# OpenDriveLab/Vista

Measured on AMD Instinct MI355X. Metric: denoise steps/sec, 25-frame 576x1024 latent, 50-step EDM @ 1/2/4/8 GPU, higher is better.
Workload: dtype bf16; 1 GPU; 1xMI355X single GPU: 25x576x1024 (latent 25x4x72x128), 50-step EulerEDM, VanillaCFG 2.5 (N=50 images per UNet call), bf16, random-init 1.65B VideoUNet, synthetic latents; frames=25, cfg_images_per_call=50, sampler=EulerEDM s_churn=0, 50-step schedule, parallelism=single GPU

## Files before the change

include/vista_hip.h:

```cpp
#ifndef VISTA_HIP_H
#define VISTA_HIP_H
#include <stdint.h>
#ifdef __cplusplus
extern "C" {
#endif

enum { VK_AMODE_DENSE = 0, VK_AMODE_CONV3X3 = 1, VK_AMODE_TEMPORAL3 = 2, VK_AMODE_CONV3D = 3 };
enum { VK_EPI_LINEAR = 0, VK_EPI_GEGLU = 1, VK_EPI_TRANS = 2 };

typedef struct VkGemmDesc {
    const void* A;
    const void* Wt;
    void* out;
    const float* bias;
    const float* rowvec;
    const void* res1;
    const void* res2;
    int32_t M, N, K;
    int32_t lda, ldc, ld_res1, ld_res2, ldv, rows_per_vec;
    float alpha, beta;
    int32_t amode, epi, out_f32;
    int32_t H, Wd, Cin, Hout, Wout, stride, ups;
    int32_t T, S;
    int32_t tile_cfg;
// ... 46 lines not shown
int vk_ff_fused_bf16(const VkGemmDesc* geglu, const VkGemmDesc* out_proj, void* stream);
int vk_ff_fused_rowstat_parts(void);

int vk_groupnorm_silu_fp8(const void* x1, const void* x2, void* y8, float* scale_out, const float* gamma, const float* beta, float* stats_ws,
                          int32_t n_img, int32_t S, int32_t C1, int32_t C2, int32_t frames_per_group, float eps, int32_t silu, void* stream);

int vk_layernorm_quant_fp8(const void* x, void* q, float* scale, const float* gamma, const float* beta, int32_t rows, int32_t C, float eps,
                           void* stream);

int vk_quantize_rows_fp8(const void* x, void* q, float* scale, int32_t M, int32_t K, int64_t ldx, int64_t ldq, void* stream);

int vk_attn_spatial_bf16(const void* q, const void* k, const void* vt, void* o, int32_t n_img, int32_t heads,
                         int32_t S, int32_t ldq, int32_t ldk, int32_t ldo, float scale, void* stream);

int vk_attn_spatial_qkv_bf16(const void* q, const void* k, const void* v, void* o, int32_t n_img, int32_t heads,
                             int32_t S, int32_t ldq, int32_t ldk, int32_t ldv, int32_t ldo, float scale, void* stream);

int vk_attn_spatial_qkv_log2_bf16(const void* q, const void* k, const void* v, void* o, int32_t n_img, int32_t heads,
                                  int32_t S, int32_t ldq, int32_t ldk, int32_t ldv, int32_t ldo, void* stream);

int vk_attn_small_bf16(const void* qkv, void* o, int32_t n_img, int32_t heads, int32_t S, int32_t D, int32_t ld, int32_t k_off,
                       int32_t v_off, int32_t ldo, float scale, void* stream);

int vk_clip_preprocess_patches(const float* img, void* out, int32_t n_img, int32_t H, int32_t W, int32_t out_hw, int32_t patch, int32_t ldo,
                               float sigma_y, float sigma_x, int32_t ks_y, int32_t ks_x, const float* mean3, const float* std3, void* stream);

int vk_attn_spatial_fp8qk(const void* q8, const void* k8, const void* q_scales, const void* k_scales, const void* v, void* o, void* o8,
                          void* o_scales, int32_t n_img, int32_t heads, int32_t S, int32_t ldq8, int32_t ldk8, int32_t ldqs, int32_t ldks,
                          int32_t ldv, int32_t ldo, int32_t ldo8, int32_t ldos, float scale, void* stream);

int vk_attn_temporal_bf16(const void* qkv, void* o, int32_t B, int32_t T, int32_t S, int32_t heads, int32_t ld,
                          int32_t k_off, int32_t v_off, int32_t ldo, float scale, void* stream);

int vk_softmax_rows_f32_bf16(const float* x, void* y, int64_t rows, int32_t cols, int64_t ldx, int64_t ldy, void* stream);

int vk_groupnorm_silu_bf16(const void* x, void* y, const float* gamma, const float* beta, float* stats_ws,
                           int32_t n_img, int32_t S, int32_t C, int32_t frames_per_group, float eps, int32_t silu,
                           void* stream);

int vk_groupnorm_stats_bf16(const void* x, float* sums, float* partial_ws, int32_t n_img, int32_t S, int32_t C,
                            int32_t frames_per_group, void* stream);
int vk_groupnorm_apply_bf16(const void* x, void* y, const float* gamma, const float* beta, const float* sums, int32_t n_img,
                            int32_t S, int32_t C, int32_t frames_per_group, float count, float eps, int32_t silu, void* stream);
int vk_groupnorm_finalize_partials(float* partial, float* sums, int32_t n_img, int32_t nchunks, int32_t frames_per_group, void* stream);
int vk_groupnorm_fold_max(void);
int vk_groupnorm_apply_partials_bf16(const void* x, void* y, const float* gamma, const float* beta, const float* partial, int32_t n_img,
                                     int32_t S, int32_t C, int32_t nchunks, int32_t frames_per_group, float count, float eps, int32_t silu,
                                     void* stream);

int vk_layernorm_bf16(const void* x, void* y, void* sum_out, const float* gamma, const float* beta,
                      const float* addvec, int32_t rows, int32_t C, int32_t rows_per_vec, int32_t ldv, float eps,
                      void* stream);

int vk_rowstats_bf16(const void* x, float* stats, int32_t rows, int32_t C, int64_t ldx, void* stream);

int vk_groupnorm_silu_cat_bf16(const void* x1, const void* x2, void* y, const float* gamma, const float* beta, float* stats_ws,
                               int32_t n_img, int32_t S, int32_t C1, int32_t C2, int32_t frames_per_group, float eps, int32_t silu,
                               void* stream);

int vk_concat_channels_bf16(const void* a, const void* b, void* out, int64_t rows, int32_t C1, int32_t C2, void* stream);

int vk_nchw_to_tokens_bf16(const float* x, void* out, int32_t n_img, int32_t C, int32_t HW, int32_t Cpad, void* stream);
int vk_tokens_to_nchw_f32(const float* x, float* out, int32_t n_img, int32_t C, int32_t HW, int32_t ldx, void* stream);

int vk_timestep_embedding_bf16(const float* t, void* out, int32_t n, int32_t dim, float max_period, void* stream);
int vk_timestep_embedding_f32(const float* t, float* out, int32_t n, int32_t dim, float max_period, void* stream);
// ... 93 lines not shown
```

vista_amd/_lib.py:

```python
import ctypes as C
import os

_HERE = os.path.dirname(os.path.abspath(__file__))
ACT_DTYPE = os.environ.get("VISTA_ACT_DTYPE", "bf16").lower()
if ACT_DTYPE not in ("bf16", "fp16"):
    raise ValueError(f"VISTA_ACT_DTYPE must be 'bf16' or 'fp16', not {ACT_DTYPE!r}")
CURRENT = ACT_DTYPE
_LIB_FILES = {"bf16": "libvista_hip.so", "fp16": "libvista_hip_f16.so"}
LIB_PATH = os.environ.get("VISTA_HIP_LIB") or os.path.join(_HERE, "lib", _LIB_FILES[ACT_DTYPE])


def lib_path(dtype_name):
    return LIB_PATH if dtype_name == ACT_DTYPE else os.path.join(_HERE, "lib", _LIB_FILES[dtype_name])


_vp = C.c_void_p
_i32 = C.c_int32
_i64 = C.c_int64
_f32 = C.c_float


class VkFp8Args(C.Structure):
    _fields_ = [("a_scale", _vp), ("w_scale", _vp), ("k_real", _i32), ("a_mx", _vp), ("ld_mx", _i32), ("mx_out", _vp), ("ld_mx_out", _i32),
                ("a_scale_rows", _i32)]
# ... 43 lines not shown

class VkStrokeSet(C.Structure):
    _fields_ = [("stroke_begin", _i32), ("stroke_count", _i32)]


class VkStrokePlan(C.Structure):
    _fields_ = [("n_sets", _i32), ("n_strokes", _i32), ("n_segments", _i32), ("reserved", _i32), ("set", VkStrokeSet * VK_OVERLAY_MAX_SETS),
                ("stroke", VkStroke * VK_OVERLAY_MAX_STROKES), ("seg", VkStrokeSegment * VK_OVERLAY_MAX_SEGMENTS)]


ABI_VERSION = 9

SIGNATURES = {
    "vk_gemm_bf16": [C.POINTER(VkGemmDesc), _vp],
    "vk_gemm_rowstat_parts": [C.POINTER(VkGemmDesc)],
    "vk_gemm_tile_choice": [C.POINTER(VkGemmDesc)],
    "vk_gemm_tail_split": [C.POINTER(VkGemmDesc)],
    "vk_gemm_gnstat_fit": [C.POINTER(VkGemmDesc)],
    "vk_gemm_fp8": [C.POINTER(VkGemmDesc), _vp, _vp, _i32, _vp],
    "vk_gemm_fp8_mx": [C.POINTER(VkGemmDesc), C.POINTER(VkFp8Args), _vp],
    "vk_gemm_fp8_rowstat_parts": [C.POINTER(VkGemmDesc)],
    "vk_ff_fused_bf16": [C.POINTER(VkGemmDesc), C.POINTER(VkGemmDesc), _vp],
    "vk_ff_fused_rowstat_parts": [],
    "vk_layernorm_quant_fp8": [_vp, _vp, _vp, _vp, _vp, _i32, _i32, _f32, _vp],
    "vk_groupnorm_silu_fp8": [_vp, _vp, _vp, _vp, _vp, _vp, _vp, _i32, _i32, _i32, _i32, _i32, _f32, _i32, _vp],
    "vk_quantize_rows_fp8": [_vp, _vp, _vp, _i32, _i32, _i64, _i64, _vp],
    "vk_attn_spatial_bf16": [_vp, _vp, _vp, _vp, _i32, _i32, _i32, _i32, _i32, _i32, _f32, _vp],
    "vk_attn_spatial_qkv_bf16": [_vp, _vp, _vp, _vp, _i32, _i32, _i32, _i32, _i32, _i32, _i32, _f32, _vp],
    "vk_attn_spatial_qkv_log2_bf16": [_vp, _vp, _vp, _vp, _i32, _i32, _i32, _i32, _i32, _i32, _i32, _vp],
    "vk_attn_spatial_fp8qk": [_vp, _vp, _vp, _vp, _vp, _vp, _vp, _vp, _i32, _i32, _i32, _i32, _i32, _i32, _i32, _i32, _i32, _i32, _i32, _f32, _vp],
    "vk_attn_small_bf16": [_vp, _vp, _i32, _i32, _i32, _i32, _i32, _i32, _i32, _i32, _f32, _vp],
    "vk_clip_preprocess_patches": [_vp, _vp, _i32, _i32, _i32, _i32, _i32, _i32, _f32, _f32, _i32, _i32, C.POINTER(_f32), C.POINTER(_f32), _vp],
    "vk_attn_temporal_bf16": [_vp, _vp, _i32, _i32, _i32, _i32, _i32, _i32, _i32, _i32, _f32, _vp],
    "vk_softmax_rows_f32_bf16": [_vp, _vp, _i64, _i32, _i64, _i64, _vp],
    "vk_groupnorm_silu_bf16": [_vp, _vp, _vp, _vp, _vp, _i32, _i32, _i32, _i32, _f32, _i32, _vp],
    "vk_groupnorm_stats_bf16": [_vp, _vp, _vp, _i32, _i32, _i32, _i32, _vp],
    "vk_groupnorm_apply_bf16": [_vp, _vp, _vp, _vp, _vp, _i32, _i32, _i32, _i32, _f32, _f32, _i32, _vp],
    "vk_groupnorm_finalize_partials": [_vp, _vp, _i32, _i32, _i32, _vp],
    "vk_groupnorm_fold_max": [],
    "vk_groupnorm_apply_partials_bf16": [_vp, _vp, _vp, _vp, _vp, _i32, _i32, _i32, _i32, _i32, _f32, _f32, _i32, _vp],
    "vk_layernorm_bf16": [_vp, _vp, _vp, _vp, _vp, _vp, _i32, _i32, _i32, _i32, _f32, _vp],
    "vk_rowstats_bf16": [_vp, _vp, _i32, _i32, _i64, _vp],
    "vk_groupnorm_silu_cat_bf16": [_vp, _vp, _vp, _vp, _vp, _vp, _i32, _i32, _i32, _i32, _i32, _f32, _i32, _vp],
    "vk_concat_channels_bf16": [_vp, _vp, _vp, _i64, _i32, _i32, _vp],
    "vk_nchw_to_tokens_bf16": [_vp, _vp, _i32, _i32, _i32, _i32, _vp],
    "vk_tokens_to_nchw_f32": [_vp, _vp, _i32, _i32, _i32, _i32, _vp],
    "vk_timestep_embedding_bf16": [_vp, _vp, _i32, _i32, _f32, _vp],
    "vk_timestep_embedding_f32": [_vp, _vp, _i32, _i32, _f32, _vp],
    "vk_emb_combine": [_vp, _vp, _vp, _vp, _vp, _vp, _i32, _i32, _vp],
    "vk_silu_f32_to_bf16": [_vp, _vp, _i64, _vp],
    "vk_cast_f32_to_bf16": [_vp, _vp, _i64, _vp],
    "vk_sampler_prepare": [_vp, _vp, _vp, _vp, _vp, _vp, _i32, _i32, _i32, _f32, _i32, _vp],
    "vk_sampler_update": [_vp, _vp, _vp, _i32, _i32, _i32, _f32, _f32, _f32, _f32, _vp],
    "vk_denoiser_combine": [_vp, _vp, _vp, _vp, _vp, _i32, _i32, _vp],
    "vk_cfg_combine": [_vp, _vp, _vp, _i32, _i32, _vp],
    "vk_euler_step": [_vp, _vp, _vp, _vp, _vp, _i32, _i32, _vp],
    "vk_mask_replace": [_vp, _vp, _vp, _vp, _i32, _i32, _vp],
    "vk_scale_rows": [_vp, _vp, _vp, _i32, _i32, _vp],
    "vk_gaussian_sample": [_vp, _vp, _vp, _i32, _i32, _i32, _f32, _vp],
    "vk_ensemble_variance_sum": [_vp, _vp, _vp, _i32, _i64, _vp],
    "vk_lanczos_resize_u8": [_vp, _vp, _vp, _vp, _vp, _i32, _vp, _vp, _i32, _vp, _i32, _i32, _i32, _i32, _i32, _i32, _i32, _i32, _i32, _vp],
    "vk_frames_to_u8": [_vp, _vp, _i32, _i32, _i32, _i32, _i32, _i32, _vp],
    "vk_ensemble_frame_stats": [_vp, _vp, _vp, _vp, _i32, _i32, _i32, _i32, _vp],
    "vk_candidate_frame_stats": [_vp, _vp, _vp, _vp, _vp, _vp, _i32, _i32, _i32, _i32, _i32, _i32, _vp],
    "vk_heat_overlay_u8": [_vp, _vp, _vp, _i32, _i32, _i32, _i32, _f32, _f32, _vp],
    "vk_frame_fidelity_ws_bytes": [_i32, _i32],
# ... 43 lines not shown
```

vista_amd/build.py:

```python
import os
import subprocess
import sys

ROOT = os.path.dirname(os.path.abspath(__file__))
REPO = os.path.dirname(ROOT)
CSRC = os.path.join(ROOT, "csrc")
LIBDIR = os.path.join(ROOT, "lib")
LIB = os.path.join(LIBDIR, "libvista_hip.so")
EXTRA_FLAGS = {"ff_fused.hip": ["-fno-slp-vectorize"], "attention.hip": ["-fno-slp-vectorize"]}
SOURCES = ["gemm.hip", "gemm_pipe.hip", "gemm_pipe2.hip", "gemm_stream.hip", "gemm_fp8.hip", "ff_fused.hip", "attention.hip", "norm.hip", "elementwise.hip", "image_io.hip", "reshard.hip", "reward.hip", "fidelity.hip", "overlay.hip"]


def hipcc():
    for c in (os.environ.get("HIPCC"), "/opt/rocm/bin/hipcc", "hipcc"):
        if c and (os.path.isabs(c) and os.path.exists(c) or not os.path.isabs(c)):
            return c
    raise RuntimeError("hipcc not found")


VARIANTS = {"bf16": ("libvista_hip.so", "", []), "fp16": ("libvista_hip_f16.so", "_f16", ["-DVK_F16=1"])}
LIB_F16 = os.path.join(LIBDIR, VARIANTS["fp16"][0])


def needs_build(lib=LIB):
    if not os.path.exists(lib):
        return True
    t = os.path.getmtime(lib)
    deps = [os.path.join(CSRC, f) for f in os.listdir(CSRC)] + [os.path.join(REPO, "include", "vista_hip.h")]
    return any(os.path.getmtime(d) > t for d in deps)


def build(force=False, verbose=True, variants=("bf16", "fp16")):
    os.makedirs(LIBDIR, exist_ok=True)
    procs, links = [], []
    for v in variants:
        libname, suffix, defs = VARIANTS[v]
        lib = os.path.join(LIBDIR, libname)
        if not force and not needs_build(lib):
            continue
        objs = []
        for s in SOURCES:
            o = os.path.join(LIBDIR, s.replace(".hip", suffix + ".o"))
            cmd = [hipcc(), "--offload-arch=gfx950", "-O3", "-std=c++17", "-fPIC", "-I" + os.path.join(REPO, "include"),
# ... 28 lines not shown
```

vista_amd/modules/diffusionmodules/sampling.py:

```python
import os
from typing import Dict, Union

import torch

from ... import ops
from ...util import append_dims, default, instantiate_from_config
from .guiders import IdentityGuider


class FusedDenoiser:

    def __init__(self, denoiser, network):
        self.denoiser, self.network = denoiser, network

    def __call__(self, x, sigma, cond, cond_mask):
        return self.denoiser(self.network, x, sigma, cond, cond_mask)


class BaseDiffusionSampler:
    def __init__(self, discretization_config: Union[Dict, None], num_steps: Union[int, None] = None,
                 guider_config: Union[Dict, None] = None, verbose: bool = False, device: str = "cuda"):
        self.num_steps = num_steps
        self.discretization = instantiate_from_config(discretization_config)
        self.guider = instantiate_from_config(default(guider_config, {"target": "vista_amd.modules.diffusionmodules.guiders.IdentityGuider"}))
# ... 146 lines not shown

    def _unet_halves(self, net_in, c_noise, graph):
        n = self.n
        half = lambda t, h: t[h * n:(h + 1) * n]
        if not graph:
            ts = torch.full((n,), c_noise, device=self.xw.device)
            return torch.cat([self.unet.forward_tokens(half(net_in, h), ts, half(self.ctx2, h), half(self.y2, h), half(self.mask2, h), self.T, self.H, self.W)
                              for h in (0, 1)])
        gs = self._graph
        if gs is None:
            gs = self._graph = [self._graph_for(half(net_in, h), n, ctx=half(self.ctx2, h), y=half(self.y2, h), mask=half(self.mask2, h), slot=h) for h in (0, 1)]
        for h in (0, 1):
            gs[h]["in"].copy_(half(net_in, h))
            gs[h]["ts"].fill_(c_noise)
        dev = net_in.device
        side = FusedLoop._CFG_STREAMS.get(dev.index)
        if side is None:
            side = FusedLoop._CFG_STREAMS[dev.index] = torch.cuda.Stream(device=dev)
        cur = torch.cuda.current_stream()
        side.wait_stream(cur)
        with torch.cuda.stream(side):
            gs[1]["graph"].replay()
        gs[0]["graph"].replay()
        cur.wait_stream(side)
        return torch.cat([gs[0]["out"], gs[1]["out"]])

    _WARM_STREAMS = {}
    _CFG_STREAMS = {}

    def _graph_for(self, net_in, n_ts, ctx=None, y=None, mask=None, slot=0):
        unet = self.unet
        cache = unet.__dict__.setdefault("_hipgraph_cache", {})
        from .. import attention as _att
        if ctx is None:
            ctx, y, mask = self.ctx2, self.y2, self.mask2
        switches = (tuple(sorted(_att.FP8.items())), _att.FF_FUSED, _att.QKV_SPLIT, _att.Q_LOG2, ops.TILE_CFG, ops.GN_EPI,
                    None if self.unet_shard is None else getattr(self.unet_shard, "a2a_chunks", None))
        key = (tuple(net_in.shape), n_ts, tuple(ctx.shape), tuple(y.shape), tuple(mask.shape), self.T, self.H, self.W,
               None if self.unet_shard is None else id(self.unet_shard), str(net_in.device), switches, slot)
        g = cache.get(key)
        wkey = (_att.pack_generation(),) + tuple((id(q), _att.Packable._param_version(q)) for q in unet.parameters())
        if g is not None and g["wkey"] != wkey:
            g = None
        if g is None:
            if ops.PROFILE_ATTN is not None:
                raise RuntimeError("ops.PROFILE_ATTN records timing events around attention launches; clear it before capturing a hipGraph")
            dev = net_in.device
            g = {"in": torch.empty_like(net_in), "ts": torch.empty((n_ts,), device=dev), "ctx": ctx.clone(), "y": y.clone(),
                 "mask": mask.clone(), "wkey": wkey}
            g["in"].copy_(net_in)
            g["ts"].fill_(0.0)
            fwd = lambda: unet.forward_tokens(g["in"], g["ts"], g["ctx"], g["y"], g["mask"], self.T, self.H, self.W, shard=self.unet_shard)
            side = FusedLoop._WARM_STREAMS.get(dev.index)
            if side is None:
                side = FusedLoop._WARM_STREAMS[dev.index] = torch.cuda.Stream(device=dev)
            with ops.graph_workspace(slot):
                side.wait_stream(torch.cuda.current_stream())
                with torch.cuda.stream(side):
                    fwd()
                torch.cuda.current_stream().wait_stream(side)
                g["wkey"] = (_att.pack_generation(),) + tuple((id(q), _att.Packable._param_version(q)) for q in unet.parameters())
                g["ws"] = ops.graph_workspace_tensor()
                g["graph"] = torch.cuda.CUDAGraph()
                mode = "global" if self.unet_shard is None else "thread_local"
                with torch.cuda.graph(g["graph"], capture_error_mode=mode):
                    g["out"] = fwd()
            cache[key] = g
        else:
            g["ctx"].copy_(ctx)
# ... 20 lines not shown
```

vista_amd/modules/video_attention.py:

```python
import torch
import torch.nn as nn

from .. import ops
from .attention import FeedForward, MemoryEfficientCrossAttention, Packable, SpatialTransformer
from .diffusionmodules.util import AlphaBlender, LayerNorm, Linear, SiLU, mlp_f32, timestep_embedding


class VideoTransformerBlock(nn.Module, Packable):
    ATTENTION_MODES = {"softmax": MemoryEfficientCrossAttention, "softmax-xformers": MemoryEfficientCrossAttention}

    def __init__(self, dim, n_heads, d_head, dropout=0.0, context_dim=None, gated_ff=True, use_checkpoint=False, timesteps=None,
                 ff_in=False, inner_dim=None, attn_mode="softmax", disable_self_attn=False, disable_temporal_crossattention=False,
                 switch_temporal_ca_to_sa=False, add_lora=False, action_control=False):
        super().__init__()
        attn_cls = self.ATTENTION_MODES[attn_mode]
        self.ff_in = ff_in or inner_dim is not None
        if inner_dim is None:
            inner_dim = dim
        assert int(n_heads * d_head) == inner_dim
        self.is_res = inner_dim == dim
        if not self.is_res:
            raise NotImplementedError("inner_dim != dim is not the Vista configuration")
        if disable_self_attn or switch_temporal_ca_to_sa:
            raise NotImplementedError("disable_self_attn / switch_temporal_ca_to_sa are not used by Vista")
        if self.ff_in:
            self.norm_in = LayerNorm(dim)
            self.ff_in = FeedForward(dim, dim_out=inner_dim, dropout=dropout, glu=gated_ff)
        self.timesteps = timesteps
        self.disable_self_attn = False
        self.attn1 = attn_cls(query_dim=inner_dim, heads=n_heads, dim_head=d_head, dropout=dropout, causal=False, add_lora=add_lora)
        self.attn1.temporal = True
        self.ff = FeedForward(inner_dim, dim_out=dim, dropout=dropout, glu=gated_ff)
        self.has_cross = not disable_temporal_crossattention
        if self.has_cross:
            self.norm2 = LayerNorm(inner_dim)
            self.attn2 = attn_cls(query_dim=inner_dim, context_dim=context_dim, heads=n_heads, dim_head=d_head, dropout=dropout,
                                  add_lora=add_lora, action_control=action_control)
        self.norm1 = LayerNorm(inner_dim)
        self.norm3 = LayerNorm(inner_dim)
        self.switch_temporal_ca_to_sa = False
        self.use_checkpoint = use_checkpoint
        self.n_heads, self.dim = n_heads, dim

    def _pack(self, dev):
        a = self.attn1
        return {"ffin_in": self.ff_in.pack_in_folded(self.norm_in, dev),
                "qkv": ops.pack_linear_cat([a.to_q.weight, a.to_k.weight, a.to_v.weight], dev, ln=self.norm1),
                "ff_in": self.ff.pack_in_folded(self.norm3, dev)}

    def forward(self, x_mix, stats, emb_rows, clip_context, B, T, S, alpha, emit_stats=False):
        assert self.timesteps is None or self.timesteps == T
        if not self.ff_in:
            raise NotImplementedError("extra_ff_mix_layer=False is not the Vista configuration")
        pk = self.packed()
        a1 = self.attn1.packed()
        x, st = self.ff_in.forward_folded(x_mix, stats, pk["ffin_in"], self.norm_in, res1=x_mix, emit_stats=True)
        qkv = ops.linear(x, pk["qkv"], ln=st, alt_cols_from=2 * x.shape[-1])
        att = ops.attn_temporal(qkv, B, T, S, self.n_heads, self.attn1.dim_head ** -0.5)
        if self.has_cross:
            cv = self.attn2.context_vector(clip_context)
            x, st = ops.linear(att, a1["out"], res1=x, rowvec=cv, rows_per_vec=T * S, emit_stats=True)
        else:
            x, st = ops.linear(att, a1["out"], res1=x, emit_stats=True)
        r = self.ff.forward_folded(x, st, pk["ff_in"], self.norm3, res1=x, alpha=1.0 - alpha, res2=x_mix, rowvec2=emb_rows.neg_rows,
                                   beta=alpha, rows_per_vec=S, emit_stats=emit_stats)
        return r if emit_stats else (r, None)


class _EmbRows:

    __slots__ = ("rows", "neg_rows")

    def __init__(self, rows):
        self.rows, self.neg_rows = rows, rows.neg()


class SpatialVideoTransformer(SpatialTransformer):

    def __init__(self, in_channels, n_heads, d_head, depth=1, dropout=0.0, use_linear=False, context_dim=None,
                 use_spatial_context=False, timesteps=None, merge_strategy="fixed", merge_factor=0.5, time_context_dim=None,
                 ff_in=False, use_checkpoint=False, time_depth=1, attn_mode="softmax", disable_self_attn=False,
                 disable_temporal_crossattention=False, max_time_embed_period=10000, add_lora=False, action_control=False):
        super().__init__(in_channels, n_heads, d_head, depth=depth, dropout=dropout, attn_type=attn_mode, use_checkpoint=use_checkpoint,
                         context_dim=context_dim, use_linear=use_linear, disable_self_attn=disable_self_attn, add_lora=add_lora,
                         action_control=action_control)
        self.time_depth = time_depth
        self.depth = depth
        self.max_time_embed_period = max_time_embed_period
        inner_dim = n_heads * d_head
        if not use_spatial_context:
            raise NotImplementedError("use_spatial_context=False (separate time_context) is not the Vista configuration")
        time_context_dim = context_dim
        self.time_stack = nn.ModuleList([
            VideoTransformerBlock(inner_dim, n_heads, d_head, dropout=dropout, context_dim=time_context_dim, timesteps=timesteps,
                                  use_checkpoint=use_checkpoint, ff_in=ff_in, inner_dim=inner_dim, attn_mode=attn_mode,
                                  disable_self_attn=disable_self_attn, disable_temporal_crossattention=disable_temporal_crossattention,
# ... 60 lines not shown
```

vista_amd/ops.py:

```python
import ctypes as C
import math
import os
import threading

import torch

from . import _lib
from ._lib import VkFp8Args, VkGemmDesc, check

AMODE_DENSE, AMODE_CONV3X3, AMODE_TEMPORAL3, AMODE_CONV3D = 0, 1, 2, 3
EPI_LINEAR, EPI_GEGLU, EPI_TRANS = 0, 1, 2
ACT = torch.float16 if _lib.ACT_DTYPE == "fp16" else torch.bfloat16
BF16 = ACT
F32 = torch.float32


class storage:

    def __init__(self, dtype):
        if dtype not in (torch.bfloat16, torch.float16):
            raise ValueError("ops.storage: torch.bfloat16 or torch.float16")
        self.dtype, self.name = dtype, ("fp16" if dtype is torch.float16 else "bf16")

    def __enter__(self):
# ... 78 lines not shown
        colsum = wt.float().sum(dim=1).contiguous()
    b = None
    if bias is not None:
        b = torch.zeros((Np,), dtype=F32, device=device)
        b[:N] = bias.to(device=device, dtype=F32)
    return PackedWeight(wt, b, ceil_to(N, 4), Kp, geglu, colsum, float(eps))


def _ln_tuple(norm):
    return (norm.weight, norm.bias, norm.eps)


KPERM16 = (0, 1, 2, 3, 8, 9, 10, 11, 4, 5, 6, 7, 12, 13, 14, 15)


def pack_linear(weight, bias=None, device="cuda", ln=None):
    return _finish_pack(weight.detach().reshape(weight.shape[0], -1).float(), None if bias is None else bias.detach().float(), device,
                        ln=None if ln is None else _ln_tuple(ln))


def ff_out_layout(w):
    N, K = w.shape
    if K % 32:
        raise ValueError("ff_out_layout needs K % 32 == 0")
    w = w.reshape(N, K // 16, 16)[:, :, list(KPERM16)].reshape(N, K // 32, 32)
    return w.permute(1, 0, 2).contiguous().reshape(K // 32 * N, 32)


def pack_ff_out(weight, bias=None, device="cuda"):
    w = weight.detach().reshape(weight.shape[0], -1).float()
    N, K = w.shape
    b = None if bias is None else bias.detach().to(device=device, dtype=F32).contiguous()
    return PackedWeight(ff_out_layout(w).to(device=device, dtype=BF16), b, N, K, ffout=True)


def pack_rows_as_weight(t, N, K):
    _need(t, BF16, "t")
    return PackedWeight(t, None, N, K)


def pack_linear_cat(weights, device="cuda", ln=None):
    return _finish_pack(torch.cat([w.detach().float() for w in weights], 0), None, device, ln=None if ln is None else _ln_tuple(ln))


def geglu_perm(nout):
    if nout % 16:
        raise ValueError("GEGLU width must be a multiple of 16")
    idx = torch.arange(nout).reshape(-1, 16)
    return torch.stack([idx, idx + nout], 1).reshape(-1)


def pack_geglu(weight, bias, device="cuda", ln=None):
    w = weight.detach().float()
    b = bias.detach().float()
    perm = geglu_perm(w.shape[0] // 2).to(w.device)
    return _finish_pack(w[perm], b[perm], device, geglu=True, ln=None if ln is None else _ln_tuple(ln))


def _slab_major(w):
    cout, taps, cin = w.shape
    return w.reshape(cout, taps, cin // 64, 64).permute(0, 2, 1, 3).reshape(cout, taps * cin)


def pack_conv3x3(weight, bias=None, cin_pad=None, device="cuda"):
    w = weight.detach().float().permute(0, 2, 3, 1).contiguous()
    cout, _, _, cin = w.shape
# ... 638 lines not shown


CLIP_MEAN = (0.48145466, 0.4578275, 0.40821073)
CLIP_STD = (0.26862954, 0.26130258, 0.27577711)


def clip_preprocess_patches(img, out_hw=224, patch=14, kpad=None, antialias=True, mean=CLIP_MEAN, std=CLIP_STD):
    _need(img, F32, "img")
    img = img.contiguous()
    n, c, H, W = img.shape
    if c != 3:
        raise ValueError("clip_preprocess_patches: 3-channel images")
    g = out_hw // patch
    kp = kpad or ceil_to(3 * patch * patch, 64)
    out = torch.zeros((n * (1 + g * g), kp), dtype=BF16, device=img.device)
    down = antialias and max(H / out_hw, W / out_hw) > 1
    (sy, ky), (sx, kx) = (antialias_blur_params(H, out_hw), antialias_blur_params(W, out_hw)) if down else ((1.0, 1), (1.0, 1))
    m3, s3 = (C.c_float * 3)(*mean), (C.c_float * 3)(*std)
    check(_lib.load().vk_clip_preprocess_patches(_p(img), _p(out), n, H, W, out_hw, patch, kp, sy, sx, ky, kx, m3, s3, _stream()),
          "vk_clip_preprocess_patches")
    return out


def attn_temporal(qkv, B, T, S, heads, scale=None):
    _need(qkv, BF16, "qkv")
    c = heads * 64
    o = torch.empty((B * T * S, c), dtype=BF16, device=qkv.device)
    lib = _lib.load()
    check(lib.vk_attn_temporal_bf16(_p(qkv), _p(o), B, T, S, heads, qkv.stride(0), c, 2 * c, o.stride(0),
                                    float(scale if scale is not None else 1.0 / math.sqrt(64)), _stream()), "vk_attn_temporal_bf16")
    return o


def softmax_rows(x, out=None):
    _need(x, F32, "x")
    rows, cols = x.shape
    if x.stride(1) != 1:
        raise ValueError("softmax_rows: rows must be contiguous")
    if out is None:
        out = torch.empty((rows, cols), dtype=BF16, device=x.device)
    check(_lib.load().vk_softmax_rows_f32_bf16(_p(x), _p(out), rows, cols, x.stride(0), out.stride(0), _stream()), "vk_softmax_rows_f32_bf16")
    return out


def _gn_partials_ok(gn, n_img, S, Cc):
    if gn is None or gn.t is None:
        return False
    if gn.rows != n_img * S or gn.C != Cc or gn.nchunks * 64 != S:
        raise ValueError(f"GnPartials of a ({gn.rows} rows, {gn.C} channels, {gn.nchunks * 64} rows per image) tensor passed to a GroupNorm over ({n_img}, {S}, {Cc})")
    return True


def groupnorm(x, gamma, beta, eps, silu, frames_per_group=1, out=None, gn=None):
    _need(x, BF16, "x")
    if not x.is_contiguous():
        raise ValueError("groupnorm: x must be contiguous")
    n_img, S, Cc = x.shape
    if out is None:
        out = torch.empty_like(x)
    if _gn_partials_ok(gn, n_img, S, Cc):
        lib = _lib.load()
        count = float(Cc // 32) * float(S) * float(frames_per_group)
        if frames_per_group * gn.nchunks <= lib.vk_groupnorm_fold_max():
            check(lib.vk_groupnorm_apply_partials_bf16(_p(x), _p(out), _p(gamma), _p(beta), _p(gn.t), n_img, S, Cc, gn.nchunks, frames_per_group, count,
                                                       float(eps), 1 if silu else 0, _stream()), "vk_groupnorm_apply_partials_bf16")
            gn.t = None
# ... 429 lines not shown
```

Baseline: 6.254 steps/s.

## Fuse temporal attention with its output projection and residual epilogue

Adds a HIP kernel that computes per-pixel temporal attention over T frames head by head and feeds each head's output straight into the out-projection GEMM via MFMA. Projection weights are streamed into LDS per head, and bias, cross-attention context rowvec, residual and row statistics are applied in the epilogue. This removes the attention output round-trip through HBM and a separate GEMM launch. It is enabled by default only for width 320 and T up to 32, so only some blocks take it, and it adds a new weight layout plus a graph-cache key switch.

```diff
diff --git a/include/vista_hip.h b/include/vista_hip.h
--- a/include/vista_hip.h
+++ b/include/vista_hip.h
@@ -102,6 +102,11 @@
 int vk_attn_temporal_bf16(const void* qkv, void* o, int32_t B, int32_t T, int32_t S, int32_t heads, int32_t ld,
                           int32_t k_off, int32_t v_off, int32_t ldo, float scale, void* stream);
 
+int vk_attn_temporal_out_bf16(const void* qkv, const VkGemmDesc* out_proj, int32_t B, int32_t T, int32_t S, int32_t heads, int32_t ld,
+                              int32_t k_off, int32_t v_off, float scale, void* stream);
+int vk_attn_temporal_out_ok(int32_t width, int32_t T);
+int vk_attn_temporal_out_rowstat_parts(int32_t width);
+
 int vk_softmax_rows_f32_bf16(const float* x, void* y, int64_t rows, int32_t cols, int64_t ldx, int64_t ldy, void* stream);
 
 int vk_groupnorm_silu_bf16(const void* x, void* y, const float* gamma, const float* beta, float* stats_ws,
diff --git a/vista_amd/_lib.py b/vista_amd/_lib.py
--- a/vista_amd/_lib.py
+++ b/vista_amd/_lib.py
@@ -99,6 +99,9 @@
     "vk_attn_small_bf16": [_vp, _vp, _i32, _i32, _i32, _i32, _i32, _i32, _i32, _i32, _f32, _vp],
     "vk_clip_preprocess_patches": [_vp, _vp, _i32, _i32, _i32, _i32, _i32, _i32, _f32, _f32, _i32, _i32, C.POINTER(_f32), C.POINTER(_f32), _vp],
     "vk_attn_temporal_bf16": [_vp, _vp, _i32, _i32, _i32, _i32, _i32, _i32, _i32, _i32, _f32, _vp],
+    "vk_attn_temporal_out_bf16": [_vp, C.POINTER(VkGemmDesc), _i32, _i32, _i32, _i32, _i32, _i32, _i32, _f32, _vp],
+    "vk_attn_temporal_out_ok": [_i32, _i32],
+    "vk_attn_temporal_out_rowstat_parts": [_i32],
     "vk_softmax_rows_f32_bf16": [_vp, _vp, _i64, _i32, _i64, _i64, _vp],
     "vk_groupnorm_silu_bf16": [_vp, _vp, _vp, _vp, _vp, _i32, _i32, _i32, _i32, _f32, _i32, _vp],
     "vk_groupnorm_stats_bf16": [_vp, _vp, _vp, _i32, _i32, _i32, _i32, _vp],
diff --git a/vista_amd/build.py b/vista_amd/build.py
--- a/vista_amd/build.py
+++ b/vista_amd/build.py
@@ -7,8 +7,9 @@
 CSRC = os.path.join(ROOT, "csrc")
 LIBDIR = os.path.join(ROOT, "lib")
 LIB = os.path.join(LIBDIR, "libvista_hip.so")
-EXTRA_FLAGS = {"ff_fused.hip": ["-fno-slp-vectorize"], "attention.hip": ["-fno-slp-vectorize"]}
-SOURCES = ["gemm.hip", "gemm_pipe.hip", "gemm_pipe2.hip", "gemm_stream.hip", "gemm_fp8.hip", "ff_fused.hip", "attention.hip", "norm.hip", "elementwise.hip", "image_io.hip", "reshard.hip", "reward.hip", "fidelity.hip", "overlay.hip"]
+EXTRA_FLAGS = {"ff_fused.hip": ["-fno-slp-vectorize"], "attention.hip": ["-fno-slp-vectorize"],
+               "attn_temporal_out.hip": ["-fno-slp-vectorize"]}
+SOURCES = ["gemm.hip", "gemm_pipe.hip", "gemm_pipe2.hip", "gemm_stream.hip", "gemm_fp8.hip", "ff_fused.hip", "attention.hip", "attn_temporal_out.hip", "norm.hip", "elementwise.hip", "image_io.hip", "reshard.hip", "reward.hip", "fidelity.hip", "overlay.hip"]
 
 
 def hipcc():
diff --git a/vista_amd/csrc/attn_temporal_out.hip b/vista_amd/csrc/attn_temporal_out.hip
--- /dev/null
+++ b/vista_amd/csrc/attn_temporal_out.hip
@@ -0,0 +1,309 @@
+#include "common.h"
+#include "vista_hip.h"
+
+#include "gemm_common.h"
+
+namespace {
+
+constexpr float TO_NEG_BIG = -1.0e30f;
+constexpr float TO_LOG2E = 1.4426950408889634f;
+constexpr int TO_NW = 320;
+constexpr int TO_NB = 10;
+
+template <int SPLIT, int NWV, bool QKL>
+__global__ __launch_bounds__(NWV * 64, 2) void attn_temporal_out_kernel(const uint16_t* __restrict__ qkv, const VkGemmDesc p,
+                                                                                          int T, int S, int ld, int k_off, int v_off,
+                                                                                          float scale_log2, long long npix) {
+    constexpr int N = TO_NW * SPLIT;
+    constexpr int HEADS = N / 64;
+    constexpr int PIX = NWV / SPLIT;
+    constexpr int CHUNK_B = N * 64;
+    constexpr int PIECES = 2 * N / 16;
+    constexpr int PPW = PIECES / NWV;
+    static_assert(PIECES % NWV == 0, "DMA pieces divide over the waves");
+    constexpr int OFF_V = 2 * CHUNK_B, OFF_BV = OFF_V + NWV * 4096;
+    constexpr int OFF_QK = OFF_BV + NWV * TO_NW * 4;
+    __shared__ __attribute__((aligned(16))) char smem[OFF_QK + (QKL ? NWV * 8192 : 0)];
+    typedef const __attribute__((address_space(1))) void* gptr_t;
+    typedef __attribute__((address_space(3))) void* lptr_t;
+
+    const int tid = threadIdx.x;
+    const int lane = tid & 63;
+    const int wave = __builtin_amdgcn_readfirstlane(tid >> 6);
+    const int l31 = lane & 31, lh = lane >> 5;
+    const int slot = wave / SPLIT, half = wave % SPLIT;
+    const int n0 = TO_NW * half;
+    char* sV = smem + OFF_V + wave * 4096;
+    float* bv = (float*)(smem + OFF_BV) + wave * TO_NW;
+    char* sQK = smem + OFF_QK + wave * 8192;
+    const bool t_ok = l31 < T;
+
+    long long pix = (long long)blockIdx.x * PIX + slot;
+    const bool active = pix < npix;
+    if (!active) pix = npix - 1;
+    const int s = (int)(pix % S);
+    const int b = (int)(pix / S);
+    const size_t row0 = (size_t)b * T * S + s;
+    const size_t rowl = row0 + (size_t)(t_ok ? l31 : 0) * S;
+
+    const uint16_t* __restrict__ Wg = (const uint16_t*)p.Wt;
+    const uint32_t dma_voff = (uint32_t)(((lane >> 2) * 32 + 8 * ((lane & 3) ^ ((lane >> 4) & 3))) * 2);
+    auto dma_head = [&](const int h) {
+#pragma unroll
+        for (int i = 0; i < PPW; ++i) {
+            const int q = wave * PPW + i;
+            const int c = q / (N / 16), rb = q % (N / 16);
+            const char* ub = (const char*)Wg + ((size_t)(2 * h + c) * N + 16 * rb) * 64;
+            __builtin_amdgcn_global_load_lds((gptr_t)(ub + dma_voff), (lptr_t)(smem + c * CHUNK_B + rb * 1024), 16, 0, 0);
+        }
+    };
+    dma_head(0);
+
+    {
+        const float* rv = p.rowvec ? p.rowvec + (size_t)(row0 / (size_t)p.rows_per_vec) * p.ldv : nullptr;
+        for (int i = lane; i < TO_NW / 4; i += 64) {
+            float4 v = make_float4(0.f, 0.f, 0.f, 0.f);
+            if (p.bias) v = *(const float4*)(p.bias + n0 + 4 * i);
+            if (rv) {
+                const float4 r = *(const float4*)(rv + n0 + 4 * i);
+                v.x += r.x; v.y += r.y; v.z += r.z; v.w += r.w;
+            }
+            *(float4*)(bv + 4 * i) = v;
+        }
+    }
+
+    f32x16_t O[TO_NB];
+    {
+        const uint16_t* __restrict__ res1 = (const uint16_t*)p.res1;
+        const uint16_t* rrow = res1 + rowl * p.ld_res1 + n0 + 8 * lh;
+#pragma unroll
+        for (int f0 = 0; f0 < TO_NB; f0 += 5) {
+            uint4 w[5][2];
+#pragma unroll
+            for (int f = 0; f < 5; ++f)
+#pragma unroll
+                for (int gp = 0; gp < 2; ++gp) w[f][gp] = res1 ? *(const uint4*)(rrow + 32 * (f0 + f) + 16 * gp) : make_uint4(0, 0, 0, 0);
+            __builtin_amdgcn_sched_barrier(0);
+#pragma unroll
+            for (int f = 0; f < 5; ++f) {
+                uint2 r1q[4];
+                unwiden_pair(w[f][0], r1q[0], r1q[1]);
+                unwiden_pair(w[f][1], r1q[2], r1q[3]);
+#pragma unroll
+                for (int g = 0; g < 4; ++g) {
+                    const uint2 r = r1q[g];
+                    O[f0 + f][4 * g + 0] = bf16_lo(r.x); O[f0 + f][4 * g + 1] = bf16_hi(r.x);
+                    O[f0 + f][4 * g + 2] = bf16_lo(r.y); O[f0 + f][4 * g + 3] = bf16_hi(r.y);
+                }
+            }
+            __builtin_amdgcn_sched_barrier(0);
+        }
+    }
+
+    const int sw = (l31 >> 2) & 3;
+    const int wrow_off = (n0 + l31) * 64;
+
+    bf16x8_t qf[4], kf[4];
+    auto load_qk = [&](const int h) {
+        const uint16_t* rp = qkv + rowl * ld + h * 64 + 8 * lh;
+#pragma unroll
+        for (int ks = 0; ks < 4; ++ks) {
+            if (QKL) {
+                if (t_ok) {
+                    __builtin_amdgcn_global_load_lds((gptr_t)(rp + 16 * ks), (lptr_t)(sQK + ks * 1024), 16, 0, 0);
+                    __builtin_amdgcn_global_load_lds((gptr_t)(rp + k_off + 16 * ks), (lptr_t)(sQK + (4 + ks) * 1024), 16, 0, 0);
+                }
+            } else {
+                uint4 a = *(const uint4*)(rp + 16 * ks);
+                uint4 c = *(const uint4*)(rp + k_off + 16 * ks);
+                if (!t_ok) { a = make_uint4(0, 0, 0, 0); c = make_uint4(0, 0, 0, 0); }
+                qf[ks] = __builtin_bit_cast(bf16x8_t, a);
+                kf[ks] = __builtin_bit_cast(bf16x8_t, c);
+            }
+        }
+    };
+    auto load_v = [&](const int h) {
+#pragma unroll
+        for (int i = 0; i < 4; ++i) {
+            const int vr = 8 * i + (lane >> 3);
+            if (vr < T)
+                __builtin_amdgcn_global_load_lds((gptr_t)(qkv + (row0 + (size_t)vr * S) * ld + v_off + h * 64 + (lane & 7) * 8), (lptr_t)(sV + i * 1024), 16, 0, 0);
+        }
+    };
+#pragma unroll
+    for (int i = 0; i < 4; ++i) *(uint4*)(sV + i * 1024 + lane * 16) = make_uint4(0, 0, 0, 0);
+    load_qk(0);
+    load_v(0);
+
+#pragma clang loop unroll(disable)
+    for (int head = 0; head < HEADS; ++head) {
+        if (QKL) {
+            __syncthreads();
+#pragma unroll
+            for (int ks = 0; ks < 4; ++ks) {
+                uint4 a = *(const uint4*)(sQK + ks * 1024 + lane * 16);
+                uint4 c = *(const uint4*)(sQK + (4 + ks) * 1024 + lane * 16);
+                if (!t_ok) { a = make_uint4(0, 0, 0, 0); c = make_uint4(0, 0, 0, 0); }
+                qf[ks] = __builtin_bit_cast(bf16x8_t, a);
+                kf[ks] = __builtin_bit_cast(bf16x8_t, c);
+            }
+        }
+        f32x16_t sacc;
+#pragma unroll
+        for (int r = 0; r < 16; ++r) sacc[r] = 0.f;
+#pragma unroll
+        for (int ks = 0; ks < 4; ++ks) sacc = vk_mfma(kf[ks], qf[ks], sacc);
+        if (QKL) {
+            asm volatile("" : "+v"(sacc));
+            if (head + 1 < HEADS) load_qk(head + 1);
+        }
+
+        float mx = TO_NEG_BIG;
+#pragma unroll
+        for (int r = 0; r < 16; ++r) {
+            const int key = (r & 3) + 8 * (r >> 2) + 4 * lh;
+            if (key >= T) sacc[r] = TO_NEG_BIG;
+            mx = fmaxf(mx, sacc[r]);
+        }
+        mx = fmaxf(mx, __shfl_xor(mx, 32, 64));
+        const float mb = mx * scale_log2;
+        float psum = 0.f;
+#pragma unroll
+        for (int r = 0; r < 16; ++r) {
+            const int key = (r & 3) + 8 * (r >> 2) + 4 * lh;
+            float pv = __builtin_amdgcn_exp2f(fmaf(sacc[r], scale_log2, -mb));
+            if (key >= T) pv = 0.f;
+            sacc[r] = pv;
+            psum += pv;
+        }
+        psum += __shfl_xor(psum, 32, 64);
+        const float inv = 1.f / psum;
+
+        bf16x8_t pf[2];
+#pragma unroll
+        for (int J = 0; J < 2; ++J) {
+            uint4 v;
+            v.x = pack_bf16x(sacc[8 * J + 0], sacc[8 * J + 1]);
+            v.y = pack_bf16x(sacc[8 * J + 2], sacc[8 * J + 3]);
+            v.z = pack_bf16x(sacc[8 * J + 4], sacc[8 * J + 5]);
+            v.w = pack_bf16x(sacc[8 * J + 6], sacc[8 * J + 7]);
+            pf[J] = __builtin_bit_cast(bf16x8_t, v);
+        }
+
+        if (!QKL) __syncthreads();
+
+        bf16x8_t hf[4];
+#pragma unroll
+        for (int d = 0; d < 2; ++d) {
+            f32x16_t oacc;
+#pragma unroll
+            for (int r = 0; r < 16; ++r) oacc[r] = 0.f;
+#pragma unroll
+            for (int J = 0; J < 2; ++J) {
+                uint32_t w[4];
+#pragma unroll
+                for (int i2 = 0; i2 < 4; ++i2) {
+                    const int ka = 16 * J + 8 * ((2 * i2) >> 2) + 4 * lh + ((2 * i2) & 3);
+                    const uint16_t lo = *(const uint16_t*)(sV + ka * 128 + (32 * d + l31) * 2);
+                    const uint16_t hi = *(const uint16_t*)(sV + (ka + 1) * 128 + (32 * d + l31) * 2);
+                    w[i2] = (uint32_t)lo | ((uint32_t)hi << 16);
+                }
+                const uint4 v = make_uint4(w[0], w[1], w[2], w[3]);
+                oacc = vk_mfma_bf16x(__builtin_bit_cast(bf16x8_t, v), pf[J], oacc);
+            }
+#pragma unroll
+            for (int gp = 0; gp < 2; ++gp) {
+                uint4 v;
+                v.x = pack_bf16(oacc[8 * gp + 0] * inv, oacc[8 * gp + 1] * inv);
+                v.y = pack_bf16(oacc[8 * gp + 2] * inv, oacc[8 * gp + 3] * inv);
+                v.z = pack_bf16(oacc[8 * gp + 4] * inv, oacc[8 * gp + 5] * inv);
+                v.w = pack_bf16(oacc[8 * gp + 6] * inv, oacc[8 * gp + 7] * inv);
+                hf[2 * d + gp] = __builtin_bit_cast(bf16x8_t, v);
+            }
+        }
+
+        if (head + 1 < HEADS) {
+            if (!QKL) load_qk(head + 1);
+            load_v(head + 1);
+        }
+
+#pragma unroll
+        for (int j = 0; j < 4; ++j) {
+            const char* ws = smem + (j >> 1) * CHUNK_B + wrow_off + (((2 * (j & 1) + lh) ^ sw) << 4);
+#pragma unroll
+            for (int f = 0; f < TO_NB; ++f) {
+                const bf16x8_t wf = *(const bf16x8_t*)(ws + f * 2048);
+                O[f] = vk_mfma(wf, hf[j], O[f]);
+            }
+        }
+
+        __syncthreads();
+        if (head + 1 < HEADS) dma_head(head + 1);
+    }
+
+    uint16_t* orow = (uint16_t*)p.out + rowl * p.ldc + n0 + 8 * lh;
+    const bool st_ok = active && t_ok;
+    float ssum = 0.f, qsum = 0.f;
+#pragma unroll
+    for (int f = 0; f < TO_NB; ++f) {
+        uint2 packed[4];
+#pragma unroll
+        for (int g = 0; g < 4; ++g) {
+            const float4 c = *(const float4*)(bv + 32 * f + 8 * g + 4 * lh);
+            packed[g].x = pack_bf16(O[f][4 * g + 0] + c.x, O[f][4 * g + 1] + c.y);
+            packed[g].y = pack_bf16(O[f][4 * g + 2] + c.z, O[f][4 * g + 3] + c.w);
+            const float a0 = bf16_lo(packed[g].x), a1 = bf16_hi(packed[g].x), a2 = bf16_lo(packed[g].y), a3 = bf16_hi(packed[g].y);
+            ssum += (a0 + a1) + (a2 + a3);
+            qsum = fmaf(a0, a0, fmaf(a1, a1, fmaf(a2, a2, fmaf(a3, a3, qsum))));
+        }
+#pragma unroll
+        for (int gp = 0; gp < 2; ++gp) {
+            const uint4 w = widen_pair(packed[2 * gp], packed[2 * gp + 1]);
+            if (st_ok) *(uint4*)(orow + 32 * f + 16 * gp) = w;
+        }
+    }
+    if (p.rowstat_out) {
+        const float so = __shfl_xor(ssum, 32, 64), qo = __shfl_xor(qsum, 32, 64);
+        if (st_ok && lh == 0) ((float2*)p.rowstat_out)[(size_t)half * p.M + rowl] = make_float2(ssum + so, qsum + qo);
+    }
+}
+
+}
+
+static bool tattn_out_takes(int width, int T) { return (width == 320 || width == 640) && T >= 1 && T <= 32; }
+
+extern "C" int vk_attn_temporal_out_ok(int32_t width, int32_t T) { return width == 320 && tattn_out_takes(width, T); }
+
+extern "C" int vk_attn_temporal_out_rowstat_parts(int32_t width) { return (width == 320 || width == 640) ? width / 320 : VK_EINVAL; }
+
+extern "C" int vk_attn_temporal_out_bf16(const void* qkv, const VkGemmDesc* d, int32_t B, int32_t T, int32_t S, int32_t heads, int32_t ld,
+                                         int32_t k_off, int32_t v_off, float scale, void* stream_) {
+    if (!qkv || !d || !d->Wt || !d->out || B <= 0 || S <= 0 || heads <= 0) return VK_EINVAL;
+    const int width = d->N;
+    if (!tattn_out_takes(width, T) || heads * 64 != width || d->K != width) return VK_EINVAL;
+    const long long M = (long long)B * T * S;
+    if (M > 0x7fffffffLL || d->M != (int)M) return VK_EINVAL;
+    if (d->amode != VK_AMODE_DENSE || d->epi != VK_EPI_LINEAR || d->out_f32 || d->A2 || d->act || d->mx8_out || d->ln_stats || d->res2 || d->rowvec2 ||
+        d->alt_cols_from || d->gnstat_out || d->alpha != 1.0f || d->m_begin || d->m_end)
+        return VK_EINVAL;
+    if ((ld % 8) != 0 || (k_off % 8) != 0 || (v_off % 8) != 0 || (((size_t)qkv) & 15) != 0 || (((size_t)d->Wt) & 15) != 0) return VK_EINVAL;
+    if (ld < width || k_off < 0 || v_off < 0) return VK_EINVAL;
+    if ((d->ldc % 8) != 0 || d->ldc < width || (((size_t)d->out) & 15) != 0) return VK_EINVAL;
+    if (d->res1 && ((d->ld_res1 % 8) != 0 || d->ld_res1 < width || (((size_t)d->res1) & 15) != 0)) return VK_EINVAL;
+    if (d->bias && (((size_t)d->bias) & 15) != 0) return VK_EINVAL;
+    if (d->rowvec && (d->rows_per_vec <= 0 || (d->rows_per_vec % ((long long)T * S)) != 0 || (d->ldv % 4) != 0 || d->ldv < width || (((size_t)d->rowvec) & 15) != 0)) return VK_EINVAL;
+    if (d->rowstat_out && (((size_t)d->rowstat_out) & 7) != 0) return VK_EINVAL;
+    const long long npix = (long long)B * S;
+    const float sl2 = scale * TO_LOG2E;
+    if (width == 320) {
+        const long long grid = (npix + 7) / 8;
+        hipLaunchKernelGGL((attn_temporal_out_kernel<1, 8, true>), dim3((unsigned)grid), dim3(512), 0, (hipStream_t)stream_, (const uint16_t*)qkv, *d, T, S, ld,
+                           k_off, v_off, sl2, npix);
+    } else {
+        const long long grid = (npix + 3) / 4;
+        hipLaunchKernelGGL((attn_temporal_out_kernel<2, 8, false>), dim3((unsigned)grid), dim3(512), 0, (hipStream_t)stream_, (const uint16_t*)qkv, *d, T, S, ld,
+                           k_off, v_off, sl2, npix);
+    }
+    VK_CHECK_LAUNCH();
+    return VK_OK;
+}
diff --git a/vista_amd/modules/diffusionmodules/sampling.py b/vista_amd/modules/diffusionmodules/sampling.py
--- a/vista_amd/modules/diffusionmodules/sampling.py
+++ b/vista_amd/modules/diffusionmodules/sampling.py
@@ -202,9 +202,10 @@
         unet = self.unet
         cache = unet.__dict__.setdefault("_hipgraph_cache", {})
         from .. import attention as _att
+        from .. import video_attention as _vatt
         if ctx is None:
             ctx, y, mask = self.ctx2, self.y2, self.mask2
-        switches = (tuple(sorted(_att.FP8.items())), _att.FF_FUSED, _att.QKV_SPLIT, _att.Q_LOG2, ops.TILE_CFG, ops.GN_EPI,
+        switches = (tuple(sorted(_att.FP8.items())), _att.FF_FUSED, _att.QKV_SPLIT, _att.Q_LOG2, _vatt.TATTN_FUSED, ops.TILE_CFG, ops.GN_EPI,
                     None if self.unet_shard is None else getattr(self.unet_shard, "a2a_chunks", None))
         key = (tuple(net_in.shape), n_ts, tuple(ctx.shape), tuple(y.shape), tuple(mask.shape), self.T, self.H, self.W,
                None if self.unet_shard is None else id(self.unet_shard), str(net_in.device), switches, slot)
diff --git a/vista_amd/modules/video_attention.py b/vista_amd/modules/video_attention.py
--- a/vista_amd/modules/video_attention.py
+++ b/vista_amd/modules/video_attention.py
@@ -1,9 +1,14 @@
+import os
+
 import torch
 import torch.nn as nn
 
 from .. import ops
 from .attention import FeedForward, MemoryEfficientCrossAttention, Packable, SpatialTransformer
 from .diffusionmodules.util import AlphaBlender, LayerNorm, Linear, SiLU, mlp_f32, timestep_embedding
+
+
+TATTN_FUSED = os.environ.get("VISTA_TATTN_FUSED", "1") != "0"
 
 
 class VideoTransformerBlock(nn.Module, Packable):
@@ -56,12 +61,20 @@
         a1 = self.attn1.packed()
         x, st = self.ff_in.forward_folded(x_mix, stats, pk["ffin_in"], self.norm_in, res1=x_mix, emit_stats=True)
         qkv = ops.linear(x, pk["qkv"], ln=st, alt_cols_from=2 * x.shape[-1])
-        att = ops.attn_temporal(qkv, B, T, S, self.n_heads, self.attn1.dim_head ** -0.5)
-        if self.has_cross:
-            cv = self.attn2.context_vector(clip_context)
-            x, st = ops.linear(att, a1["out"], res1=x, rowvec=cv, rows_per_vec=T * S, emit_stats=True)
+        scale = self.attn1.dim_head ** -0.5
+        if TATTN_FUSED and self.attn1.dim_head == 64 and ops.attn_temporal_out_ok(x.shape[-1], T):
+            if "out_tattn" not in a1:
+                a1["out_tattn"] = ops.pack_tattn_out(self.attn1.to_out[0].weight, self.attn1.to_out[0].bias, x.device)
+            cv = self.attn2.context_vector(clip_context) if self.has_cross else None
+            x, st = ops.attn_temporal_out(qkv, a1["out_tattn"], B, T, S, self.n_heads, scale, res1=x, rowvec=cv,
+                                          rows_per_vec=T * S if cv is not None else 0, emit_stats=True)
         else:
-            x, st = ops.linear(att, a1["out"], res1=x, emit_stats=True)
+            att = ops.attn_temporal(qkv, B, T, S, self.n_heads, scale)
+            if self.has_cross:
+                cv = self.attn2.context_vector(clip_context)
+                x, st = ops.linear(att, a1["out"], res1=x, rowvec=cv, rows_per_vec=T * S, emit_stats=True)
+            else:
+                x, st = ops.linear(att, a1["out"], res1=x, emit_stats=True)
         r = self.ff.forward_folded(x, st, pk["ff_in"], self.norm3, res1=x, alpha=1.0 - alpha, res2=x_mix, rowvec2=emb_rows.neg_rows,
                                    beta=alpha, rows_per_vec=S, emit_stats=emit_stats)
         return r if emit_stats else (r, None)
diff --git a/vista_amd/ops.py b/vista_amd/ops.py
--- a/vista_amd/ops.py
+++ b/vista_amd/ops.py
@@ -134,6 +134,28 @@
     N, K = w.shape
     b = None if bias is None else bias.detach().to(device=device, dtype=F32).contiguous()
     return PackedWeight(ff_out_layout(w).to(device=device, dtype=BF16), b, N, K, ffout=True)
+
+
+def tattn_out_layout(w):
+    N, K = w.shape
+    if K % 64:
+        raise ValueError("tattn_out_layout needs K % 64 == 0 (whole heads)")
+    w = w.reshape(N, K // 16, 16)[:, :, list(KPERM16)].reshape(N, K // 32, 32)
+    return w.permute(1, 0, 2).contiguous().reshape(K // 32 * N, 32)
+
+
+def tattn_out_layout_inverse(wp, N):
+    K = wp.numel() // N
+    inv = [KPERM16.index(i) for i in range(16)]
+    w = wp.reshape(K // 32, N, 32).permute(1, 0, 2).reshape(N, K // 16, 16)[:, :, inv]
+    return w.reshape(N, K).contiguous()
+
+
+def pack_tattn_out(weight, bias=None, device="cuda"):
+    w = weight.detach().reshape(weight.shape[0], -1).float()
+    N, K = w.shape
+    b = None if bias is None else bias.detach().to(device=device, dtype=F32).contiguous()
+    return PackedWeight(tattn_out_layout(w).to(device=device, dtype=BF16), b, N, K, ffout=True)
 
 
 def pack_rows_as_weight(t, N, K):
@@ -838,6 +860,36 @@
     return o
 
 
+def attn_temporal_out_ok(width, T):
+    return bool(_lib.load().vk_attn_temporal_out_ok(int(width), int(T)))
+
+
+def attn_temporal_out(qkv, pw_out, B, T, S, heads, scale=None, *, res1, rowvec=None, rows_per_vec=0, emit_stats=True, out=None, stats_out=None):
+    _need(qkv, BF16, "qkv")
+    c = heads * 64
+    M = B * T * S
+    if not pw_out.ffout or pw_out.N != c or pw_out.K != c or qkv.dim() != 2 or qkv.shape[0] != M or qkv.shape[1] != 3 * c or qkv.stride(1) != 1:
+        raise ValueError("attn_temporal_out: needs qkv ((b t) s, 3*heads*64) and a pack_tattn_out weight [heads*64][heads*64]")
+    if out is None:
+        out = torch.empty((M, c), dtype=BF16, device=qkv.device)
+    d = VkGemmDesc()
+    d.A, d.lda = _p(qkv), qkv.stride(0)
+    d.amode, d.epi = AMODE_DENSE, EPI_LINEAR
+    _fill_epilogue(d, pw_out, out, M, rowvec, rows_per_vec, res1, None, 1.0, 0.0)
+    lib = _lib.load()
+    stats = None
+    if emit_stats:
+        parts = lib.vk_attn_temporal_out_rowstat_parts(c)
+        if parts <= 0:
+            raise _lib.VistaHipError(f"vk_attn_temporal_out_rowstat_parts failed with code {parts}")
+        t = stats_out if stats_out is not None else torch.empty((parts, M, 2), dtype=F32, device=qkv.device)
+        stats = RowStats(t, parts, M)
+        d.rowstat_out = _p(t)
+    check(lib.vk_attn_temporal_out_bf16(_p(qkv), C.byref(d), B, T, S, heads, qkv.stride(0), c, 2 * c,
+                                        float(scale if scale is not None else 1.0 / math.sqrt(64)), _stream()), "vk_attn_temporal_out_bf16")
+    return (out, stats) if emit_stats else out
+
+
 def softmax_rows(x, out=None):
     _need(x, F32, "x")
     rows, cols = x.shape
```

New measurement: 6.281 steps/s, median of 6. About the same (+0.4%).
